# CogSP/CoEvoNet

Measured on AMD Instinct MI355X. Metric: env-steps/sec (agent-steps of the whole job; generations/sec in gens_per_sec), Co-GA simple_adversary_v3 pop=200 HoF=5, higher is better.
Workload: dtype f32

## Files before the change

coevonet_amd/csrc/philox.hip.h:

```cpp
#pragma once
#include "coevo_common.hip.h"

namespace coevo {

struct u32x4 { uint32_t v[4]; };

constexpr int COEVO_NOISE_ROUNDS = 7;

template <int ROUNDS>
__device__ inline u32x4 philox4x32(uint32_t c0, uint32_t c1, uint32_t c2, uint32_t c3, uint32_t k0, uint32_t k1)
{
#pragma unroll
    for (int r = 0; r < ROUNDS; ++r) {
        const uint64_t p0 = (uint64_t)0xD2511F53u * c0, p1 = (uint64_t)0xCD9E8D57u * c2;
        const uint32_t n0 = (uint32_t)(p1 >> 32) ^ c1 ^ k0, n1 = (uint32_t)p1;
        const uint32_t n2 = (uint32_t)(p0 >> 32) ^ c3 ^ k1, n3 = (uint32_t)p0;
        c0 = n0; c1 = n1; c2 = n2; c3 = n3;
        k0 += 0x9E3779B9u; k1 += 0xBB67AE85u;
    }
    return u32x4{{c0, c1, c2, c3}};
}

__device__ inline u32x4 philox4x32_10(uint32_t c0, uint32_t c1, uint32_t c2, uint32_t c3, uint32_t k0, uint32_t k1)
{
    return philox4x32<10>(c0, c1, c2, c3, k0, k1);
}

__device__ inline float canon_logf(float x)
{
    const uint32_t b = __float_as_uint(x);
    int e = (int)((b >> 23) & 0xff) - 126;
    float m = __uint_as_float((b & 0x007fffffu) | 0x3f000000u);
    if (m < 0.707106781186547524f) { e -= 1; m = (m + m) - 1.0f; } else { m = m - 1.0f; }
    const float z = m * m;
    float y = 7.0376836292E-2f;
    y = __builtin_fmaf(y, m, -1.1514610310E-1f);
    y = __builtin_fmaf(y, m, 1.1676998740E-1f);
    y = __builtin_fmaf(y, m, -1.2420140846E-1f);
    y = __builtin_fmaf(y, m, 1.4249322787E-1f);
    y = __builtin_fmaf(y, m, -1.6668057665E-1f);
    y = __builtin_fmaf(y, m, 2.0000714765E-1f);
    y = __builtin_fmaf(y, m, -2.4999993993E-1f);
    y = __builtin_fmaf(y, m, 3.3333331174E-1f);
    y = (y * m) * z;
    const float fe = (float)e;
    y = __builtin_fmaf(-2.12194440e-4f, fe, y);
    y = __builtin_fmaf(-0.5f, z, y);
    float r = m + y;
    r = __builtin_fmaf(0.693359375f, fe, r);
    return r;
}

__device__ inline void canon_sincos2pi(float u, float &c_out, float &s_out)
{
    const float t = u * 4.0f;
    const float qf = __builtin_floorf(t);
    const int q = (int)qf;
    float f = t - qf;
    const bool swap = f > 0.5f;
    if (swap) f = 1.0f - f;
    const float x = f * 1.57079632679489661923f;
    const float z = x * x;
    float sp = -1.9515295891E-4f;
    sp = __builtin_fmaf(sp, z, 8.3321608736E-3f);
    sp = __builtin_fmaf(sp, z, -1.6666654611E-1f);
    float s = __builtin_fmaf(sp * z, x, x);
    float cp = 2.443315711809948E-005f;
    cp = __builtin_fmaf(cp, z, -1.388731625493765E-003f);
    cp = __builtin_fmaf(cp, z, 4.166664568298827E-002f);
    float c = __builtin_fmaf(cp * z, z, __builtin_fmaf(-0.5f, z, 1.0f));
    if (swap) { const float tmp = s; s = c; c = tmp; }
    switch (q & 3) {
    case 0: c_out = c; s_out = s; break;
    case 1: c_out = -s; s_out = c; break;
    case 2: c_out = -c; s_out = -s; break;
    default: c_out = s; s_out = -c; break;
    }
}

__device__ inline void box_muller(uint32_t a, uint32_t b, float &z0, float &z1)
{
    const float u1 = (float)(2u * (a >> 9) + 1u) * 5.9604644775390625e-08f;
    const float u2 = (float)(b >> 8) * 5.9604644775390625e-08f;
    const float r = __builtin_sqrtf(-2.0f * canon_logf(u1));
    float c, s;
    canon_sincos2pi(u2, c, s);
    z0 = r * c;
    z1 = r * s;
}

__device__ inline void philox_normal4(uint64_t seed, uint32_t stream_lo, uint32_t stream_hi, uint32_t q, float z[4])
{
    const u32x4 o = philox4x32<COEVO_NOISE_ROUNDS>(q, stream_lo, stream_hi, 0x636f6576u, (uint32_t)seed, (uint32_t)(seed >> 32));
    box_muller(o.v[0], o.v[1], z[0], z[1]);
    box_muller(o.v[2], o.v[3], z[2], z[3]);
}

}
```

Before: 149.3 million.

## Vectorize Box-Muller noise generation with packed f32x2 math and bit-trick log/sincos

```diff
diff --git a/coevonet_amd/csrc/philox.hip.h b/coevonet_amd/csrc/philox.hip.h
--- a/coevonet_amd/csrc/philox.hip.h
+++ b/coevonet_amd/csrc/philox.hip.h
@@ -7,93 +7,134 @@
 
 constexpr int COEVO_NOISE_ROUNDS = 7;
 
+__host__ __device__ inline uint32_t xor3(uint32_t a, uint32_t b, uint32_t c)
+{
+#if defined(__HIP_DEVICE_COMPILE__)
+    return __builtin_amdgcn_bitop3_b32(a, b, c, 0x96);
+#else
+    return a ^ b ^ c;
+#endif
+}
+
 template <int ROUNDS>
-__device__ inline u32x4 philox4x32(uint32_t c0, uint32_t c1, uint32_t c2, uint32_t c3, uint32_t k0, uint32_t k1)
+__host__ __device__ inline u32x4 philox4x32(uint32_t c0, uint32_t c1, uint32_t c2, uint32_t c3, uint32_t k0, uint32_t k1)
 {
 #pragma unroll
     for (int r = 0; r < ROUNDS; ++r) {
         const uint64_t p0 = (uint64_t)0xD2511F53u * c0, p1 = (uint64_t)0xCD9E8D57u * c2;
-        const uint32_t n0 = (uint32_t)(p1 >> 32) ^ c1 ^ k0, n1 = (uint32_t)p1;
-        const uint32_t n2 = (uint32_t)(p0 >> 32) ^ c3 ^ k1, n3 = (uint32_t)p0;
+        const uint32_t n0 = r > 1 ? xor3((uint32_t)(p1 >> 32), c1, k0) : (uint32_t)(p1 >> 32) ^ c1 ^ k0, n1 = (uint32_t)p1;
+        const uint32_t n2 = r > 1 ? xor3((uint32_t)(p0 >> 32), c3, k1) : (uint32_t)(p0 >> 32) ^ c3 ^ k1, n3 = (uint32_t)p0;
         c0 = n0; c1 = n1; c2 = n2; c3 = n3;
         k0 += 0x9E3779B9u; k1 += 0xBB67AE85u;
     }
     return u32x4{{c0, c1, c2, c3}};
 }
 
-__device__ inline u32x4 philox4x32_10(uint32_t c0, uint32_t c1, uint32_t c2, uint32_t c3, uint32_t k0, uint32_t k1)
+__host__ __device__ inline u32x4 philox4x32_10(uint32_t c0, uint32_t c1, uint32_t c2, uint32_t c3, uint32_t k0, uint32_t k1)
 {
     return philox4x32<10>(c0, c1, c2, c3, k0, k1);
 }
 
-__device__ inline float canon_logf(float x)
+typedef float f32x2 __attribute__((ext_vector_type(2)));
+typedef uint32_t u32x2 __attribute__((ext_vector_type(2)));
+typedef int32_t i32x2 __attribute__((ext_vector_type(2)));
+
+__host__ __device__ inline f32x2 fma2(f32x2 a, f32x2 b, f32x2 c) { return __builtin_elementwise_fma(a, b, c); }
+__host__ __device__ inline f32x2 splat2(float v) { return f32x2{v, v}; }
+__host__ __device__ inline f32x2 u2f_bits(u32x2 b) { return __builtin_bit_cast(f32x2, b); }
+__host__ __device__ inline u32x2 f2u_bits(f32x2 f) { return __builtin_bit_cast(u32x2, f); }
+__host__ __device__ inline f32x2 u2f_value(u32x2 n) { return f32x2{(float)n[0], (float)n[1]}; }
+
+__host__ __device__ inline f32x2 canon_logf2(u32x2 n256)
 {
-    const uint32_t b = __float_as_uint(x);
-    int e = (int)((b >> 23) & 0xff) - 126;
-    float m = __uint_as_float((b & 0x007fffffu) | 0x3f000000u);
-    if (m < 0.707106781186547524f) { e -= 1; m = (m + m) - 1.0f; } else { m = m - 1.0f; }
-    const float z = m * m;
-    float y = 7.0376836292E-2f;
-    y = __builtin_fmaf(y, m, -1.1514610310E-1f);
-    y = __builtin_fmaf(y, m, 1.1676998740E-1f);
-    y = __builtin_fmaf(y, m, -1.2420140846E-1f);
-    y = __builtin_fmaf(y, m, 1.4249322787E-1f);
-    y = __builtin_fmaf(y, m, -1.6668057665E-1f);
-    y = __builtin_fmaf(y, m, 2.0000714765E-1f);
-    y = __builtin_fmaf(y, m, -2.4999993993E-1f);
-    y = __builtin_fmaf(y, m, 3.3333331174E-1f);
+    const u32x2 ix = f2u_bits(u2f_value(n256)) + (0x3f800000u - 0x3f3504f3u - (32u << 23) - (127u << 23));
+    const f32x2 fe = f32x2{(float)((int32_t)ix[0] >> 23), (float)((int32_t)ix[1] >> 23)};
+    const f32x2 m = u2f_bits((ix & 0x007fffffu) + 0x3f3504f3u) + splat2(-1.0f);
+    const f32x2 z = m * m;
+    f32x2 y = splat2(7.0376836292E-2f);
+    y = fma2(y, m, splat2(-1.1514610310E-1f));
+    y = fma2(y, m, splat2(1.1676998740E-1f));
+    y = fma2(y, m, splat2(-1.2420140846E-1f));
+    y = fma2(y, m, splat2(1.4249322787E-1f));
+    y = fma2(y, m, splat2(-1.6668057665E-1f));
+    y = fma2(y, m, splat2(2.0000714765E-1f));
+    y = fma2(y, m, splat2(-2.4999993993E-1f));
+    y = fma2(y, m, splat2(3.3333331174E-1f));
     y = (y * m) * z;
-    const float fe = (float)e;
-    y = __builtin_fmaf(-2.12194440e-4f, fe, y);
-    y = __builtin_fmaf(-0.5f, z, y);
-    float r = m + y;
-    r = __builtin_fmaf(0.693359375f, fe, r);
+    y = fma2(splat2(-2.12194440e-4f), fe, y);
+    y = fma2(splat2(-0.5f), z, y);
+    f32x2 r = m + y;
+    r = fma2(splat2(0.693359375f), fe, r);
     return r;
 }
 
-__device__ inline void canon_sincos2pi(float u, float &c_out, float &s_out)
+__host__ __device__ inline f32x2 canon_sqrt_fixup2(f32x2 x, f32x2 s)
 {
-    const float t = u * 4.0f;
-    const float qf = __builtin_floorf(t);
-    const int q = (int)qf;
-    float f = t - qf;
-    const bool swap = f > 0.5f;
-    if (swap) f = 1.0f - f;
-    const float x = f * 1.57079632679489661923f;
-    const float z = x * x;
-    float sp = -1.9515295891E-4f;
-    sp = __builtin_fmaf(sp, z, 8.3321608736E-3f);
-    sp = __builtin_fmaf(sp, z, -1.6666654611E-1f);
-    float s = __builtin_fmaf(sp * z, x, x);
-    float cp = 2.443315711809948E-005f;
-    cp = __builtin_fmaf(cp, z, -1.388731625493765E-003f);
-    cp = __builtin_fmaf(cp, z, 4.166664568298827E-002f);
-    float c = __builtin_fmaf(cp * z, z, __builtin_fmaf(-0.5f, z, 1.0f));
-    if (swap) { const float tmp = s; s = c; c = tmp; }
-    switch (q & 3) {
-    case 0: c_out = c; s_out = s; break;
-    case 1: c_out = -s; s_out = c; break;
-    case 2: c_out = -c; s_out = -s; break;
-    default: c_out = s; s_out = -c; break;
+    const f32x2 dn = u2f_bits(f2u_bits(s) - 1u), up = u2f_bits(f2u_bits(s) + 1u);
+    const f32x2 e_dn = fma2(-dn, s, x), e_up = fma2(-up, s, x);
+    f32x2 r;
+#pragma unroll
+    for (int i = 0; i < 2; ++i) {
+        r[i] = e_dn[i] <= 0.0f ? dn[i] : s[i];
+        r[i] = e_up[i] > 0.0f ? up[i] : r[i];
     }
+    return r;
 }
 
-__device__ inline void box_muller(uint32_t a, uint32_t b, float &z0, float &z1)
+__host__ __device__ inline f32x2 canon_sqrtf2(f32x2 x)
 {
-    const float u1 = (float)(2u * (a >> 9) + 1u) * 5.9604644775390625e-08f;
-    const float u2 = (float)(b >> 8) * 5.9604644775390625e-08f;
-    const float r = __builtin_sqrtf(-2.0f * canon_logf(u1));
-    float c, s;
-    canon_sincos2pi(u2, c, s);
-    z0 = r * c;
-    z1 = r * s;
+#if defined(__HIP_DEVICE_COMPILE__)
+    return canon_sqrt_fixup2(x, f32x2{__builtin_amdgcn_sqrtf(x[0]), __builtin_amdgcn_sqrtf(x[1])});
+#else
+    return canon_sqrt_fixup2(x, f32x2{__builtin_sqrtf(x[0]), __builtin_sqrtf(x[1])});
+#endif
 }
 
-__device__ inline void philox_normal4(uint64_t seed, uint32_t stream_lo, uint32_t stream_hi, uint32_t q, float z[4])
+__host__ __device__ inline void canon_sincos2pi2(u32x2 b, f32x2 &c_out, f32x2 &s_out)
+{
+    const u32x2 j = (b >> 8) & 0x003fffffu;
+    u32x2 jf;
+#pragma unroll
+    for (int i = 0; i < 2; ++i) jf[i] = j[i] < 0x00400000u - j[i] ? j[i] : 0x00400000u - j[i];
+    const f32x2 x = u2f_value(jf) * splat2(1.57079632679489661923f * 2.384185791015625e-07f);
+    const f32x2 z = x * x;
+    f32x2 sp = splat2(-1.9515295891E-4f);
+    sp = fma2(sp, z, splat2(8.3321608736E-3f));
+    sp = fma2(sp, z, splat2(-1.6666654611E-1f));
+    const f32x2 s = fma2(sp * z, x, x);
+    f32x2 cp = splat2(2.443315711809948E-005f);
+    cp = fma2(cp, z, splat2(-1.388731625493765E-003f));
+    cp = fma2(cp, z, splat2(4.166664568298827E-002f));
+    const f32x2 c = fma2(cp * z, z, fma2(splat2(-0.5f), z, splat2(1.0f)));
+    const u32x2 su = f2u_bits(s), cu = f2u_bits(c);
+    const u32x2 sign_c = b + 0x40000000u;
+    u32x2 co, so;
+#pragma unroll
+    for (int i = 0; i < 2; ++i) {
+        const bool keep = (int32_t)((b[i] << 1) - (0x00200001u << 9)) < 0;
+        const uint32_t cm = keep ? cu[i] : su[i], sm = keep ? su[i] : cu[i];
+        co[i] = (cm & 0x7fffffffu) | (sign_c[i] & 0x80000000u);
+        so[i] = (sm & 0x7fffffffu) | (b[i] & 0x80000000u);
+    }
+    c_out = u2f_bits(co);
+    s_out = u2f_bits(so);
+}
+
+__host__ __device__ inline void box_muller2(u32x2 a, u32x2 b, f32x2 &za, f32x2 &zb)
+{
+    const f32x2 r = canon_sqrtf2(splat2(-2.0f) * canon_logf2((a & 0xffffff00u) | 0x100u));
+    f32x2 c, s;
+    canon_sincos2pi2(b, c, s);
+    za = f32x2{r[0], r[0]} * f32x2{c[0], s[0]};
+    zb = f32x2{r[1], r[1]} * f32x2{c[1], s[1]};
+}
+
+__host__ __device__ inline void philox_normal4(uint64_t seed, uint32_t stream_lo, uint32_t stream_hi, uint32_t q, float z[4])
 {
     const u32x4 o = philox4x32<COEVO_NOISE_ROUNDS>(q, stream_lo, stream_hi, 0x636f6576u, (uint32_t)seed, (uint32_t)(seed >> 32));
-    box_muller(o.v[0], o.v[1], z[0], z[1]);
-    box_muller(o.v[2], o.v[3], z[2], z[3]);
+    f32x2 za, zb;
+    box_muller2(u32x2{o.v[0], o.v[2]}, u32x2{o.v[1], o.v[3]}, za, zb);
+    z[0] = za[0]; z[1] = za[1]; z[2] = zb[0]; z[3] = zb[1];
 }
 
 }
```

New measurement: 150.6 million (median of 6 runs). No clear change (+0.8%).
